# arkiven4/glow-tts

Measured on AMD Instinct MI355X. Metric: mel_frames_per_sec_train_step, higher is better.
Workload: dtype bf16; 1 GPU; configs/base.json, LJSpeech-shaped synthetic batches, B=32/GPU, T_x<=150, T_y<=800, bf16 GEMMs; batch_per_gpu=32, T_x=150, T_y=800, batches_rotated=8, padded_frames_per_gpu_step=25600, rows_layout=ragged, graphs_captured=6, parallelism=dp1 (utterance-sharded, RCCL gradient all-reduce, fp32 on the wire), launch=one HIP graph per step (one per ragged-row bucket, captured up front)

## Files before the change

### glow-tts_amd/csrc/conv_wgrad.hip

```cpp
#include <stdlib.h>
#include "common.h"
#include "mfma_frag.h"
#include "../../include/glowtts_hip.h"

namespace {

constexpr int SLAB_Q = 64;

typedef __attribute__((__vector_size__(4 * sizeof(short)))) short s16x4_t;

__device__ __forceinline__ unsigned lds_off(const void* p) { return (unsigned)reinterpret_cast<uintptr_t>(p); }

__device__ __forceinline__ bf16x8_t tr_frag(const unsigned char* p0, const unsigned char* p1) {
  const s16x4_t lo = __builtin_amdgcn_ds_read_tr16_b64_v4i16((__attribute__((address_space(3))) s16x4_t*)(uintptr_t)p0);
  const s16x4_t hi = __builtin_amdgcn_ds_read_tr16_b64_v4i16((__attribute__((address_space(3))) s16x4_t*)(uintptr_t)p1);
  typedef __attribute__((__vector_size__(8 * sizeof(short)))) short s16x8_t;
  s16x8_t v = {lo[0], lo[1], lo[2], lo[3], hi[0], hi[1], hi[2], hi[3]};
  return __builtin_bit_cast(bf16x8_t, v);
}

__device__ __forceinline__ void glds16(const void* src, unsigned dst_base) {
  unsigned keep;
  asm volatile("s_mov_b32 %0, m0\n\ts_mov_b32 m0, %2\n\ts_nop 0\n\t"
               "global_load_lds_dwordx4 %1, off\n\ts_mov_b32 m0, %0"
               : "=&s"(keep) : "v"(src), "s"(dst_base) : "memory");
}
template <int N> __device__ __forceinline__ void wait_vm() { asm volatile("s_waitcnt vmcnt(%0)" :: "n"(N) : "memory"); }

template <int TAPS, int NJ, int KB_, int NST_> struct WgGeo {
  static constexpr int KB = KB_, NST = NST_;
  static constexpr int XR = KB + TAPS - 1;
  static constexpr int XCH = 8 * NJ;
  static constexpr int YB = KB * 256, XB = XR * XCH * 16, STAGE = YB + XB;
  static constexpr int YI = KB / 16;
  static constexpr int NWX = XR * XCH / 4;
  static constexpr int XI = (NWX + 63) / 64;
  static constexpr int NLD = YI + XI;
  static constexpr int NB = TAPS * NJ;
  static constexpr int LDS = NST * STAGE;
  static_assert(KB % 16 == 0 && SLAB_Q % KB == 0, "stage rows");
  static_assert((XR * XCH) % 4 == 0, "X chunks split evenly over the waves");
  static_assert(LDS <= 80 * 1024, "two workgroups per CU");
  static_assert((NST - 2) * NLD <= 63, "vmcnt field");
  static_assert(TAPS == 1 || NJ == 1, "taps or channel groups");
};

template <int TAPS, int NJ, int KB_, int NST_>
__device__ __forceinline__ void wgrad_tile(
    const bf16_t* __restrict__ X, int ldx, const bf16_t* __restrict__ dY, int ldy,
    float* __restrict__ part, float* __restrict__ part_bias, int R, int Cin, int Cout, int slab_rows,
    int co0, int ci0, int slab, int co_begin, int Ncols)
{
  using G = WgGeo<TAPS, NJ, KB_, NST_>;
  constexpr int KB = G::KB, NST = G::NST, NB = G::NB;
  extern __shared__ __attribute__((aligned(1024))) unsigned char ring[];
  const int tid = threadIdx.x, lane = tid & 63, wave = __builtin_amdgcn_readfirstlane(tid >> 6);
  constexpr int padl = TAPS >> 1;
  const int mbeg = slab * slab_rows;
  const int mend = min(R, mbeg + slab_rows);
  const int nst = (mend - mbeg + KB - 1) / KB;
  const int wco = wave >> 1, wci = wave & 1;
  const bool do_bias = (ci0 == 0) && part_bias && wci == 0;

  f32x16_t acc[NB][2];
  float bsum[2] = {0.f, 0.f};
#pragma unroll
  for (int t = 0; t < NB; ++t)
#pragma unroll
    for (int j = 0; j < 2; ++j)
#pragma unroll
      for (int e = 0; e < 16; ++e) acc[t][j][e] = 0.0f;

  int yrow[G::YI], ycol[G::YI], xrow[G::XI], xcol[G::XI];
  bool xact[G::XI];
#pragma unroll
  for (int j = 0; j < G::YI; ++j) {
    const int L = j * 256 + tid, r = L >> 4, c = (L & 15) ^ ((r & 3) << 2);
    yrow[j] = r; ycol[j] = min(co0 + c * 8, Ncols - 8);
  }
#pragma unroll
  for (int j = 0; j < G::XI; ++j) {
    const int Lw = j * 64 + lane, L = wave * G::NWX + Lw, r = L / G::XCH, c = (L - r * G::XCH) ^ (((r >> 1) & 1) << 2);
    xact[j] = Lw < G::NWX;
    xrow[j] = r - padl; xcol[j] = min(ci0 + c * 8, Cin - 8);
  }
  const unsigned ring0 = lds_off(ring);

  auto issue = [&](int s, int sl_i) {
    const int mb = mbeg + s * KB;
    const unsigned slot = ring0 + (unsigned)sl_i * G::STAGE;
    const bool edge = (mb - padl < 0) || (mb + KB + padl > R) || (mb + KB > mend);
    if (!edge) {
#pragma unroll
      for (int j = 0; j < G::YI; ++j)
        glds16(dY + (size_t)(mb + yrow[j]) * ldy + ycol[j], slot + (unsigned)(j * 256 + wave * 64) * 16);
#pragma unroll
      for (int j = 0; j < G::XI; ++j)
        if (xact[j]) glds16(X + (ptrdiff_t)(mb + xrow[j]) * ldx + xcol[j], slot + G::YB + (unsigned)(wave * G::NWX + j * 64) * 16);
    } else {
      unsigned char* sl = ring + (size_t)sl_i * G::STAGE;
#pragma unroll
      for (int j = 0; j < G::YI; ++j) {
        const int m = mb + yrow[j];
        u32x4_t v = {0u, 0u, 0u, 0u};
        if (m < mend) v = *reinterpret_cast<const u32x4_t*>(dY + (size_t)m * ldy + ycol[j]);
        *reinterpret_cast<u32x4_t*>(sl + (size_t)(j * 256 + tid) * 16) = v;
      }
#pragma unroll
      for (int j = 0; j < G::XI; ++j) {
        const int m = mb + xrow[j];
        u32x4_t v = {0u, 0u, 0u, 0u};
        if (xact[j]) {
          if (m >= 0 && m < R) v = *reinterpret_cast<const u32x4_t*>(X + (size_t)m * ldx + xcol[j]);
          *reinterpret_cast<u32x4_t*>(sl + G::YB + (size_t)(wave * G::NWX + j * 64 + lane) * 16) = v;
        }
      }
    }
  };

  const int li = lane & 15, q = li >> 2, p = li & 3;
  const int colhalf = ((lane >> 4) & 1) * 16;
  const int h = lane >> 5;
  constexpr int NOX = TAPS < 4 ? TAPS : 4;
  int offA[2], offX[NOX];
#pragma unroll
  for (int i = 0; i < 2; ++i) {
    const int ch = wco * 8 + i * 4 + (colhalf >> 3) + (p >> 1);
    offA[i] = (8 * h + q) * 256 + ((ch ^ (q << 2)) << 4) + (p & 1) * 8;
  }
#pragma unroll
  for (int t = 0; t < NOX; ++t) {
    const int ch = wci * 4 + (colhalf >> 3) + (p >> 1);
    offX[t] = (8 * h + q) * (G::XCH * 16) + ((ch ^ ((((q + t) >> 1) & 1) << 2)) << 4) + (p & 1) * 8;
  }

  bf16x8_t af[2], bfg[NB];
  auto load_frags = [&](const unsigned char* yb, const unsigned char* xb, int ks) {
#pragma unroll
    for (int i = 0; i < 2; ++i) {
      const unsigned char* ya = yb + offA[i] + ks * 16 * 256;
      af[i] = tr_frag(ya, ya + 4 * 256);
    }
#pragma unroll
    for (int t = 0; t < TAPS; ++t)
#pragma unroll
      for (int j = 0; j < NJ; ++j) {
        const unsigned char* xa = xb + offX[t & 3] + (ks * 16 + t) * (G::XCH * 16) + j * 128;
        bfg[t * NJ + j] = tr_frag(xa, xa + 4 * (G::XCH * 16));
      }
  };
  auto mfmas = [&]() {
#pragma unroll
    for (int t = 0; t < NB; ++t)
#pragma unroll
      for (int i = 0; i < 2; ++i) acc[t][i] = __builtin_amdgcn_mfma_f32_32x32x16_bf16(af[i], bfg[t], acc[t][i], 0, 0, 0);
    if (do_bias) {
#pragma unroll
      for (int i = 0; i < 2; ++i) {
        const u32x4_t w4 = __builtin_bit_cast(u32x4_t, af[i]);
#pragma unroll
        for (int d = 0; d < 4; ++d) bsum[i] += __uint_as_float(w4[d] << 16) + __uint_as_float(w4[d] & 0xffff0000u);
      }
    }
  };

#pragma unroll 1
  for (int s = 0; s < NST - 1 && s < nst; ++s) issue(s, s);
  int cslot = 0, islot = NST - 1;
#pragma unroll 1
  for (int s = 0; s < nst; ++s) {
    const int after = min(nst - 1, s + NST - 2) - s;
    if (after >= NST - 2) wait_vm<(NST - 2) * G::NLD>();
    else wait_vm<0>();
    asm volatile("s_waitcnt lgkmcnt(0)\n\ts_barrier" ::: "memory");
    if (s + NST - 1 < nst) issue(s + NST - 1, islot);
    const unsigned char* yb = ring + (size_t)cslot * G::STAGE;
    const unsigned char* xb = yb + G::YB;
    cslot = cslot + 1 == NST ? 0 : cslot + 1;
    islot = islot + 1 == NST ? 0 : islot + 1;
#pragma unroll
    for (int ks = 0; ks < KB / 16; ++ks) {
      load_frags(yb, xb, ks);
      __builtin_amdgcn_sched_barrier(0);
      mfmas();
    }
  }

  const int r = lane & 31;
#pragma unroll
  for (int t = 0; t < TAPS; ++t)
#pragma unroll
    for (int j = 0; j < NJ; ++j) {
      const int ci = ci0 + j * 64 + wci * 32 + r;
#pragma unroll
      for (int i = 0; i < 2; ++i) {
        if (ci >= Cin) continue;
#pragma unroll
        for (int e = 0; e < 16; ++e) {
          const int co = co0 + wco * 64 + i * 32 + (e & 3) + 8 * (e >> 2) + 4 * h;
          if (co < Ncols) part[(((size_t)slab * TAPS + t) * Cout + co_begin + co) * Cin + ci] = acc[t * NJ + j][i][e];
        }
      }
    }
  if (do_bias) {
#pragma unroll
    for (int i = 0; i < 2; ++i) {
      const float tot = bsum[i] + __shfl_xor(bsum[i], 32);
      const int co = co0 + wco * 64 + i * 32 + r;
      if (h == 0 && co < Ncols) part_bias[(size_t)slab * Cout + co_begin + co] = tot;
    }
  }
}

template <int TAPS> struct WgSel;
template <> struct WgSel<5> { static constexpr int NJ = 1, KB = 64, NST = 3; };
template <> struct WgSel<3> { static constexpr int NJ = 1, KB = 64, NST = 3; };
template <> struct WgSel<1> { static constexpr int NJ = 3, KB = 32, NST = 3; };
template <int TAPS> using WgGeoT = WgGeo<TAPS, WgSel<TAPS>::NJ, WgSel<TAPS>::KB, WgSel<TAPS>::NST>;

template <int TAPS>
__global__ __launch_bounds__(256, 2) void gt_conv_wgrad_kernel(
    const bf16_t* __restrict__ X, int ldx, const bf16_t* __restrict__ dY, int ldy,
    float* __restrict__ part, float* __restrict__ part_bias, int R, int Cin, int Cout, int slab_rows)
{
  using S = WgSel<TAPS>;
  wgrad_tile<TAPS, S::NJ, S::KB, S::NST>(X, ldx, dY, ldy, part, part_bias, R, Cin, Cout, slab_rows,
                                         blockIdx.x * 128, blockIdx.y * 64 * S::NJ, blockIdx.z, 0, Cout);
}

template <int TAPS>
__global__ __launch_bounds__(256, 2) void gt_conv_wgrad_batched_kernel(
    const gt_wgrad_job* __restrict__ jobs, const gt_wgrad_tile* __restrict__ tiles)
{
  using S = WgSel<TAPS>;
  const gt_wgrad_tile t = tiles[blockIdx.x];
  const gt_wgrad_job j = jobs[t.job];
  wgrad_tile<TAPS, S::NJ, S::KB, S::NST>(static_cast<const bf16_t*>(j.X), j.ldx, static_cast<const bf16_t*>(j.dY), j.ldy,
                                         j.part, j.part_bias, j.R, j.Cin, j.Cout, j.slab_rows, t.co0, t.ci0, t.slab, j.co_begin, j.co_count);
}

template <int TAPS> static int wgrad_lds_attr()
{
  static int done = 0;
  if (!done) {
    if (hipFuncSetAttribute(reinterpret_cast<const void*>(&gt_conv_wgrad_kernel<TAPS>), hipFuncAttributeMaxDynamicSharedMemorySize, WgGeoT<TAPS>::LDS) != hipSuccess ||
        hipFuncSetAttribute(reinterpret_cast<const void*>(&gt_conv_wgrad_batched_kernel<TAPS>), hipFuncAttributeMaxDynamicSharedMemorySize, WgGeoT<TAPS>::LDS) != hipSuccess)
      return GT_E_LAUNCH;
    done = 1;
  }
  return 0;
}

constexpr int WNB_ROWS = 4;
__device__ __forceinline__ void weightnorm_bwd_row(
    const float* __restrict__ part, const float* __restrict__ part_bias, int S, const float* __restrict__ v,
    const float* __restrict__ g, const float* __restrict__ inv_norm, float* __restrict__ dv, float* __restrict__ dg,
    float* __restrict__ dbias, int Cout, int Cin, int taps, int accumulate, int co, float* dws)
{
  const int lane = threadIdx.x & 63, n = Cin * taps;
  if (dbias && lane == 0) {
    float sb = 0.f;
    for (int k = 0; k < S; ++k) sb += part_bias[(size_t)k * Cout + co];
    dbias[co] = accumulate ? dbias[co] + sb : sb;
  }
  const size_t sstride = (size_t)taps * Cout * Cin;
  for (int tap = 0; tap < taps; ++tap) {
    const float* pt = part + ((size_t)tap * Cout + co) * Cin;
    for (int ci = lane; ci < Cin; ci += 64) {
      const float* pp = pt + ci;
      float s0 = 0.f, s1 = 0.f, s2 = 0.f, s3 = 0.f;
      int k = 0;
      for (; k + 4 <= S; k += 4) {
        const float a0 = pp[(size_t)k * sstride], a1 = pp[(size_t)(k + 1) * sstride];
        const float a2 = pp[(size_t)(k + 2) * sstride], a3 = pp[(size_t)(k + 3) * sstride];
        s0 += a0; s1 += a1; s2 += a2; s3 += a3;
      }
      for (; k < S; ++k) s0 += pp[(size_t)k * sstride];
      dws[ci * taps + tap] = (s0 + s1) + (s2 + s3);
    }
  }
  __builtin_amdgcn_fence(__ATOMIC_RELEASE, "wavefront");
  __builtin_amdgcn_wave_barrier();
  __builtin_amdgcn_fence(__ATOMIC_ACQUIRE, "wavefront");
  const float* vr = v + (size_t)co * n;
  float* dr = dv + (size_t)co * n;
  if (!g) {
    for (int i = lane; i < n; i += 64) dr[i] = accumulate ? dr[i] + dws[i] : dws[i];
    return;
  }
  float dot = 0.f;
  for (int i = lane; i < n; i += 64) dot += dws[i] * vr[i];
  const float d = wave_sum(dot);
  const float inv = inv_norm[co], gg = g[co];
  if (lane == 0) dg[co] = accumulate ? dg[co] + d * inv : d * inv;
  const float a = gg * inv, bcoef = gg * d * inv * inv * inv;
  for (int i = lane; i < n; i += 64) {
    const float val = a * dws[i] - bcoef * vr[i];
    dr[i] = accumulate ? dr[i] + val : val;
  }
}

__global__ __launch_bounds__(64 * WNB_ROWS) void gt_weightnorm_bwd_kernel(
    const float* __restrict__ part, const float* __restrict__ part_bias, int S, const float* __restrict__ v,
    const float* __restrict__ g, const float* __restrict__ inv_norm, float* __restrict__ dv, float* __restrict__ dg,
    float* __restrict__ dbias, int Cout, int Cin, int taps, int accumulate)
{
  extern __shared__ float dws[];
  const int w = threadIdx.x >> 6, co = blockIdx.x * WNB_ROWS + w;
  if (co >= Cout) return;
  weightnorm_bwd_row(part, part_bias, S, v, g, inv_norm, dv, dg, dbias, Cout, Cin, taps, accumulate, co, dws + (size_t)w * Cin * taps);
}

__global__ __launch_bounds__(64 * WNB_ROWS) void gt_weightnorm_bwd_batched_kernel(const gt_wnb_job* __restrict__ jobs, int n_jobs, int total_rows,
                                                                                int max_row_elems)
{
  extern __shared__ float dws[];
  const int w = threadIdx.x >> 6, row = blockIdx.x * WNB_ROWS + w;
  if (row >= total_rows) return;
  int lo = 0, hi = n_jobs - 1;
  while (lo < hi) {
    const int mid = (lo + hi + 1) >> 1;
    if (jobs[mid].row_start <= row) lo = mid; else hi = mid - 1;
  }
  const gt_wnb_job j = jobs[lo];
  weightnorm_bwd_row(j.part, j.part_bias, j.S, j.v, j.g, j.inv_norm, j.dv, j.dg, j.dbias, j.Cout, j.Cin, j.taps,
                     j.accumulate, row - j.row_start, dws + (size_t)w * max_row_elems);
}

template <bool F32>
__global__ __launch_bounds__(256) void gt_colsum_kernel(const void* __restrict__ Y, int ldy, float* __restrict__ out,
                                                        int R, int N, int rows_per_block)
{
  __shared__ float red[4][64];
  const int c = blockIdx.x * 64 + (threadIdx.x & 63), ph = threadIdx.x >> 6;
  const int m0 = blockIdx.y * rows_per_block, m1 = min(R, m0 + rows_per_block);
  float s = 0.f;
  if (c < N) {
    for (int m = m0 + ph; m < m1; m += 4)
      s += F32 ? static_cast<const float*>(Y)[(size_t)m * ldy + c] : bf2f(static_cast<const bf16_t*>(Y)[(size_t)m * ldy + c]);
  }
  red[ph][threadIdx.x & 63] = s;
  __syncthreads();
  if (ph == 0 && c < N) atomicAdd(out + c, red[0][threadIdx.x] + red[1][threadIdx.x] + red[2][threadIdx.x] + red[3][threadIdx.x]);
}

}

extern "C" int gt_conv_wgrad_ci_tile(int taps)
{
  return taps == 1 ? 64 * WgSel<1>::NJ : taps == 3 ? 64 * WgSel<3>::NJ : taps == 5 ? 64 * WgSel<5>::NJ : 0;
}

extern "C" size_t gt_conv_wgrad_workspace_bytes(int R, int Cin, int Cout, int taps, int* slabs_out)
{
  if (R <= 0 || Cin <= 0 || Cout <= 0 || taps <= 0) { if (slabs_out) *slabs_out = 0; return 0; }
  const int cit = gt_conv_wgrad_ci_tile(taps) > 0 ? gt_conv_wgrad_ci_tile(taps) : 64;
  const int tiles = ((Cout + 127) / 128) * ((Cin + cit - 1) / cit);
  constexpr int target = 160;
  int S = (target + tiles - 1) / tiles;
  if (S > 16) S = 16;
  const int max_s = (R + SLAB_Q - 1) / SLAB_Q;
  if (S > max_s) S = max_s;
  if (S < 1) S = 1;
  if (slabs_out) *slabs_out = S;
  return ((size_t)S * taps * Cout * Cin + (size_t)S * Cout) * sizeof(float);
}

extern "C" int gt_conv_wgrad_bf16(const void* X, int ldx, const void* dY, int ldy, int R, int Cin, int Cout,
                                  int taps, void* workspace, size_t workspace_bytes, void* stream)
{
  if (R <= 0 || Cin <= 0 || Cout <= 0) return GT_E_INVAL;
  if (!X || !dY || !workspace) return GT_E_INVAL;
  if (taps != 1 && taps != 3 && taps != 5) return GT_E_UNSUPPORTED;
  if ((Cin & 7) || (Cout & 7) || (ldx & 7) || (ldy & 7)) return GT_E_ALIGN;
  if (((uintptr_t)X | (uintptr_t)dY) & 15) return GT_E_ALIGN;
  int S = 0;
  if (workspace_bytes < gt_conv_wgrad_workspace_bytes(R, Cin, Cout, taps, &S)) return GT_E_INVAL;
  const int slab_rows = (((R + S - 1) / S) + SLAB_Q - 1) / SLAB_Q * SLAB_Q;
  const int cit = gt_conv_wgrad_ci_tile(taps);
  const dim3 grid((Cout + 127) / 128, (Cin + cit - 1) / cit, S);
  hipStream_t st = static_cast<hipStream_t>(stream);
  const bf16_t* x = static_cast<const bf16_t*>(X); const bf16_t* dy = static_cast<const bf16_t*>(dY);
  float* part = static_cast<float*>(workspace);
  float* pb = part + (size_t)S * taps * Cout * Cin;
  if (wgrad_lds_attr<5>() || wgrad_lds_attr<3>() || wgrad_lds_attr<1>()) return GT_E_LAUNCH;
  if (taps == 5)      hipLaunchKernelGGL(gt_conv_wgrad_kernel<5>, grid, dim3(256), WgGeoT<5>::LDS, st, x, ldx, dy, ldy, part, pb, R, Cin, Cout, slab_rows);
  else if (taps == 3) hipLaunchKernelGGL(gt_conv_wgrad_kernel<3>, grid, dim3(256), WgGeoT<3>::LDS, st, x, ldx, dy, ldy, part, pb, R, Cin, Cout, slab_rows);
  else                hipLaunchKernelGGL(gt_conv_wgrad_kernel<1>, grid, dim3(256), WgGeoT<1>::LDS, st, x, ldx, dy, ldy, part, pb, R, Cin, Cout, slab_rows);
  return gt_launch_status(__func__);
}

extern "C" int gt_weightnorm_bwd(const void* workspace, int R, const float* v, const float* g, const float* inv_norm,
                                 float* dv, float* dg, float* dbias, int Cout, int Cin, int taps, int accumulate, void* stream)
{
  if (!workspace || !v || !dv || Cout <= 0 || Cin <= 0 || taps <= 0) return GT_E_INVAL;
  if (g && (!inv_norm || !dg)) return GT_E_INVAL;
  int S = 0;
  gt_conv_wgrad_workspace_bytes(R, Cin, Cout, taps, &S);
  const size_t lds = (size_t)WNB_ROWS * Cin * taps * sizeof(float);
  if (lds > 60 * 1024) return GT_E_UNSUPPORTED;
  const float* part = static_cast<const float*>(workspace);
  hipLaunchKernelGGL(gt_weightnorm_bwd_kernel, dim3((Cout + WNB_ROWS - 1) / WNB_ROWS), dim3(64 * WNB_ROWS), lds, static_cast<hipStream_t>(stream),
                     part, part + (size_t)S * taps * Cout * Cin, S, v, g, inv_norm, dv, dg, dbias, Cout, Cin, taps, accumulate);
  return gt_launch_status(__func__);
}

extern "C" int gt_conv_wgrad_batched(const void* jobs_device, const void* tiles_device, int n_tiles5, int n_tiles3,
                                     int n_tiles1, void* stream)
{
  if (!jobs_device || !tiles_device || n_tiles5 < 0 || n_tiles3 < 0 || n_tiles1 < 0) return GT_E_INVAL;
  hipStream_t st = static_cast<hipStream_t>(stream);
  const gt_wgrad_job* jobs = static_cast<const gt_wgrad_job*>(jobs_device);
  const gt_wgrad_tile* tiles = static_cast<const gt_wgrad_tile*>(tiles_device);
  if (wgrad_lds_attr<5>() || wgrad_lds_attr<3>() || wgrad_lds_attr<1>()) return GT_E_LAUNCH;
  if (n_tiles5) hipLaunchKernelGGL(gt_conv_wgrad_batched_kernel<5>, dim3(n_tiles5), dim3(256), WgGeoT<5>::LDS, st, jobs, tiles);
  if (n_tiles3) hipLaunchKernelGGL(gt_conv_wgrad_batched_kernel<3>, dim3(n_tiles3), dim3(256), WgGeoT<3>::LDS, st, jobs, tiles + n_tiles5);
  if (n_tiles1) hipLaunchKernelGGL(gt_conv_wgrad_batched_kernel<1>, dim3(n_tiles1), dim3(256), WgGeoT<1>::LDS, st, jobs, tiles + n_tiles5 + n_tiles3);
  return gt_launch_status(__func__);
}

extern "C" int gt_weightnorm_bwd_batched(const void* jobs_device, int n_jobs, int total_rows, int max_row_elems, void* stream)
{
  if (!jobs_device || n_jobs <= 0 || total_rows <= 0 || max_row_elems <= 0) return GT_E_INVAL;
  const size_t lds = (size_t)WNB_ROWS * max_row_elems * sizeof(float);
  if (lds > 60 * 1024) return GT_E_UNSUPPORTED;
  hipLaunchKernelGGL(gt_weightnorm_bwd_batched_kernel, dim3((total_rows + WNB_ROWS - 1) / WNB_ROWS), dim3(64 * WNB_ROWS), lds,
                     static_cast<hipStream_t>(stream), static_cast<const gt_wnb_job*>(jobs_device), n_jobs, total_rows, max_row_elems);
  return gt_launch_status(__func__);
}

extern "C" int gt_colsum(const void* Y, int ldy, int is_f32, float* out, int R, int N, void* stream)
{
  if (!Y || !out || R < 0 || N <= 0) return GT_E_INVAL;
  if (R == 0) return GT_OK;
  const int rows_per_block = 128;
  const dim3 grid((N + 63) / 64, (R + rows_per_block - 1) / rows_per_block);
  hipStream_t st = static_cast<hipStream_t>(stream);
  if (is_f32) hipLaunchKernelGGL(gt_colsum_kernel<true>,  grid, dim3(256), 0, st, Y, ldy, out, R, N, rows_per_block);
  else        hipLaunchKernelGGL(gt_colsum_kernel<false>, grid, dim3(256), 0, st, Y, ldy, out, R, N, rows_per_block);
  return gt_launch_status(__func__);
}
```

Before: 4.493 million mel-frames/s.

## Vectorize weight-norm backward with float4 slab reduction and LDS-staged v

Adds a wide path for the weight-norm backward row kernel. It sums split-K partial slabs with 16-byte vector loads using several accumulators, and stages both the reduced weight gradient and the v row in LDS, so the dot product and the dv update read LDS instead of global memory. The bias reduction switches to shuffles, and the batched kernel finds the job with a ballot/popcount scan instead of a binary search. LDS per row doubles, so the rows per block are now chosen dynamically to stay under the LDS cap, which can lower the number of rows per block and the occupancy for large rows.

```diff
diff --git a/glow-tts_amd/csrc/conv_wgrad.hip b/glow-tts_amd/csrc/conv_wgrad.hip
--- a/glow-tts_amd/csrc/conv_wgrad.hip
+++ b/glow-tts_amd/csrc/conv_wgrad.hip
@@ -300,31 +300,211 @@
   }
 }
 
-__global__ __launch_bounds__(64 * WNB_ROWS) void gt_weightnorm_bwd_kernel(
+constexpr int WNF_P = 4;
+typedef float wnf4_t __attribute__((ext_vector_type(4)));
+__device__ __forceinline__ wnf4_t wnf_ld4(const float* p) { return *(const __attribute__((address_space(1))) wnf4_t*)(uintptr_t)p; }
+__device__ __forceinline__ float wnf_ld1(const float* p) { return *(const __attribute__((address_space(1))) float*)(uintptr_t)p; }
+__device__ __forceinline__ void wnf_st4(float* p, wnf4_t x) { *(__attribute__((address_space(1))) wnf4_t*)(uintptr_t)p = x; }
+
+__device__ __forceinline__ float wnf_dv(float a, float dw, float bcoef, float x)
+{
+#pragma clang fp contract(off)
+  const float l = a * dw, r = bcoef * x;
+  return l - r;
+}
+
+template <int NS>
+__device__ __forceinline__ void wnf_slabs_few(const float* const (&pp)[WNF_P], size_t sstride, wnf4_t (&t)[WNF_P])
+{
+  asm volatile("; %0 slab(s) per pass" :: "n"(NS) : "memory");
+  wnf4_t a[WNF_P][NS];
+#pragma unroll
+  for (int p = 0; p < WNF_P; ++p)
+#pragma unroll
+    for (int q = 0; q < NS; ++q) a[p][q] = wnf_ld4(pp[p] + (size_t)q * sstride);
+#pragma unroll
+  for (int p = 0; p < WNF_P; ++p) {
+    wnf4_t s0 = 0.f;
+#pragma unroll
+    for (int q = 0; q < NS; ++q) s0 += a[p][q];
+    t[p] = (s0 + 0.f) + (0.f + 0.f);
+  }
+}
+
+__device__ __forceinline__ void weightnorm_bwd_row16(
+    const float* __restrict__ part, const float* __restrict__ part_bias, int S, const float* __restrict__ v,
+    const float* __restrict__ g, const float* __restrict__ inv_norm, float* __restrict__ dv, float* __restrict__ dg,
+    float* __restrict__ dbias, int Cout, int Cin, int taps, int accumulate, int co, float* dws, float* vs)
+{
+  const int lane = threadIdx.x & 63, n = Cin * taps, nch = n >> 2;
+  const unsigned c4 = (unsigned)Cin >> 2;
+  const size_t sstride = (size_t)taps * Cout * Cin;
+  const float* vr = v + (size_t)co * n;
+  float* dr = dv + (size_t)co * n;
+  float pb, odb, inv, gg, odg;
+  if (dbias) {
+    pb = wnf_ld1(part_bias + (size_t)max(min(lane, S - 1), 0) * Cout + co);
+    if (accumulate) odb = wnf_ld1(dbias + co);
+  }
+  if (g) {
+    inv = wnf_ld1(inv_norm + co); gg = wnf_ld1(g + co);
+    if (accumulate) odg = wnf_ld1(dg + co);
+  }
+  wnf4_t od[WNF_P];
+  if (accumulate) {
+#pragma unroll
+    for (int p = 0; p < WNF_P; ++p) od[p] = wnf_ld4(dr + 4 * min(64 * p + lane, nch - 1));
+  }
+  for (int c0 = 0; c0 < nch; c0 += 64 * WNF_P) {
+    const float* pp[WNF_P]; int o[WNF_P]; wnf4_t vv[WNF_P], t[WNF_P];
+#pragma unroll
+    for (int p = 0; p < WNF_P; ++p) {
+      const unsigned c = (unsigned)min(c0 + 64 * p + lane, nch - 1);
+      const unsigned tap = c / c4, ci = (c - tap * c4) * 4;
+      pp[p] = part + ((size_t)tap * Cout + co) * Cin + ci;
+      o[p] = (int)(ci * taps + tap);
+    }
+    if (g) {
+#pragma unroll
+      for (int p = 0; p < WNF_P; ++p) vv[p] = wnf_ld4(vr + 4 * min(c0 + 64 * p + lane, nch - 1));
+    }
+    if (S <= 2) {
+      if (S == 1) wnf_slabs_few<1>(pp, sstride, t);
+      else        wnf_slabs_few<2>(pp, sstride, t);
+#pragma unroll
+      for (int p = 0; p < WNF_P; ++p) {
+        if (c0 + 64 * p + lane >= nch) continue;
+        float* d = dws + o[p];
+        d[0] = t[p].x; d[taps] = t[p].y; d[2 * taps] = t[p].z; d[3 * taps] = t[p].w;
+      }
+    } else {
+#pragma unroll 1
+      for (int p = 0; p < WNF_P; ++p) {
+        const int cp = c0 + 64 * p + lane;
+        const unsigned c = (unsigned)min(cp, nch - 1);
+        const unsigned tap = c / c4, ci = (c - tap * c4) * 4;
+        const float* q = part + ((size_t)tap * Cout + co) * Cin + ci;
+        wnf4_t s0 = 0.f, s1 = 0.f, s2 = 0.f, s3 = 0.f;
+        int k = 0;
+        for (; k + 4 <= S; k += 4) {
+          const wnf4_t a0 = wnf_ld4(q + (size_t)k * sstride), a1 = wnf_ld4(q + (size_t)(k + 1) * sstride);
+          const wnf4_t a2 = wnf_ld4(q + (size_t)(k + 2) * sstride), a3 = wnf_ld4(q + (size_t)(k + 3) * sstride);
+          s0 += a0; s1 += a1; s2 += a2; s3 += a3;
+        }
+        for (; k < S; ++k) s0 += wnf_ld4(q + (size_t)k * sstride);
+        const wnf4_t r = (s0 + s1) + (s2 + s3);
+        if (cp < nch) {
+          float* d = dws + ci * taps + tap;
+          d[0] = r.x; d[taps] = r.y; d[2 * taps] = r.z; d[3 * taps] = r.w;
+        }
+      }
+    }
+    if (g) {
+#pragma unroll
+      for (int p = 0; p < WNF_P; ++p) {
+        const int c = c0 + 64 * p + lane;
+        if (c < nch) *reinterpret_cast<wnf4_t*>(vs + 4 * c) = vv[p];
+      }
+    }
+  }
+  if (dbias) {
+    float sb = 0.f;
+    for (int k0 = 0; k0 < S; k0 += 64) {
+      if (k0) pb = wnf_ld1(part_bias + (size_t)min(k0 + lane, S - 1) * Cout + co);
+      const int m = min(64, S - k0);
+      for (int k = 0; k < m; ++k) sb += __shfl(pb, k);
+    }
+    if (lane == 0) dbias[co] = accumulate ? odb + sb : sb;
+  }
+  __builtin_amdgcn_fence(__ATOMIC_RELEASE, "wavefront");
+  __builtin_amdgcn_wave_barrier();
+  __builtin_amdgcn_fence(__ATOMIC_ACQUIRE, "wavefront");
+  float a = 1.f, bcoef = 0.f;
+  if (g) {
+    float dot = 0.f;
+    for (int i = lane; i < n; i += 64) dot = __builtin_fmaf(dws[i], vs[i], dot);
+    const float d = wave_sum(dot);
+    if (lane == 0) dg[co] = accumulate ? __builtin_fmaf(d, inv, odg) : d * inv;
+    a = gg * inv; bcoef = gg * d * inv * inv * inv;
+  }
+  for (int c0 = 0; c0 < nch; c0 += 64 * WNF_P) {
+    if (c0 && accumulate) {
+#pragma unroll
+      for (int p = 0; p < WNF_P; ++p) od[p] = wnf_ld4(dr + 4 * min(c0 + 64 * p + lane, nch - 1));
+    }
+#pragma unroll
+    for (int p = 0; p < WNF_P; ++p) {
+      const int c = c0 + 64 * p + lane;
+      if (c >= nch) continue;
+      wnf4_t val = *reinterpret_cast<const wnf4_t*>(dws + 4 * c);
+      if (g) {
+        const wnf4_t x = *reinterpret_cast<const wnf4_t*>(vs + 4 * c);
+        val.x = wnf_dv(a, val.x, bcoef, x.x); val.y = wnf_dv(a, val.y, bcoef, x.y);
+        val.z = wnf_dv(a, val.z, bcoef, x.z); val.w = wnf_dv(a, val.w, bcoef, x.w);
+      }
+      if (accumulate) { val.x = od[p].x + val.x; val.y = od[p].y + val.y; val.z = od[p].z + val.z; val.w = od[p].w + val.w; }
+      wnf_st4(dr + 4 * c, val);
+    }
+  }
+}
+
+__device__ __forceinline__ void weightnorm_bwd_dispatch(
+    const float* __restrict__ part, const float* __restrict__ part_bias, int S, const float* __restrict__ v,
+    const float* __restrict__ g, const float* __restrict__ inv_norm, float* __restrict__ dv, float* __restrict__ dg,
+    float* __restrict__ dbias, int Cout, int Cin, int taps, int accumulate, int co, float* strip, int strip_elems)
+{
+  const bool wide = !(Cin & 3) && !((reinterpret_cast<uintptr_t>(part) | reinterpret_cast<uintptr_t>(v) | reinterpret_cast<uintptr_t>(dv)) & 15);
+  if (wide) {
+    weightnorm_bwd_row16(part, part_bias, S, v, g, inv_norm, dv, dg, dbias, Cout, Cin, taps, accumulate, co, strip, strip + strip_elems);
+  } else {
+    weightnorm_bwd_row(part, part_bias, S, v, g, inv_norm, dv, dg, dbias, Cout, Cin, taps, accumulate, co, strip);
+    __builtin_amdgcn_s_waitcnt(0x0070);
+  }
+}
+
+__global__ __launch_bounds__(64 * WNB_ROWS, 3) void gt_weightnorm_bwd_kernel(
     const float* __restrict__ part, const float* __restrict__ part_bias, int S, const float* __restrict__ v,
     const float* __restrict__ g, const float* __restrict__ inv_norm, float* __restrict__ dv, float* __restrict__ dg,
     float* __restrict__ dbias, int Cout, int Cin, int taps, int accumulate)
 {
-  extern __shared__ float dws[];
-  const int w = threadIdx.x >> 6, co = blockIdx.x * WNB_ROWS + w;
+  extern __shared__ __attribute__((aligned(16))) float dws[];
+  const int w = threadIdx.x >> 6, co = blockIdx.x * (blockDim.x >> 6) + w;
   if (co >= Cout) return;
-  weightnorm_bwd_row(part, part_bias, S, v, g, inv_norm, dv, dg, dbias, Cout, Cin, taps, accumulate, co, dws + (size_t)w * Cin * taps);
-}
-
-__global__ __launch_bounds__(64 * WNB_ROWS) void gt_weightnorm_bwd_batched_kernel(const gt_wnb_job* __restrict__ jobs, int n_jobs, int total_rows,
+  const int strip = (Cin * taps + 3) & ~3;
+  weightnorm_bwd_dispatch(part, part_bias, S, v, g, inv_norm, dv, dg, dbias, Cout, Cin, taps, accumulate, co, dws + (size_t)w * 2 * strip, strip);
+}
+
+__global__ __launch_bounds__(64 * WNB_ROWS, 3) void gt_weightnorm_bwd_batched_kernel(const gt_wnb_job* __restrict__ jobs, int n_jobs, int total_rows,
                                                                                 int max_row_elems)
 {
-  extern __shared__ float dws[];
-  const int w = threadIdx.x >> 6, row = blockIdx.x * WNB_ROWS + w;
+  extern __shared__ __attribute__((aligned(16))) float dws[];
+  const int w = threadIdx.x >> 6, lane = threadIdx.x & 63, row = blockIdx.x * (blockDim.x >> 6) + w;
   if (row >= total_rows) return;
-  int lo = 0, hi = n_jobs - 1;
-  while (lo < hi) {
-    const int mid = (lo + hi + 1) >> 1;
-    if (jobs[mid].row_start <= row) lo = mid; else hi = mid - 1;
-  }
+  int cnt = 0;
+  for (int i0 = 0; i0 < n_jobs; i0 += 256) {
+    int rs[4];
+#pragma unroll
+    for (int u = 0; u < 4; ++u) {
+      const int i = i0 + 64 * u + lane;
+      rs[u] = jobs[min(i, n_jobs - 1)].row_start;
+    }
+#pragma unroll
+    for (int u = 0; u < 4; ++u) cnt += __popcll(__ballot(i0 + 64 * u + lane < n_jobs && rs[u] <= row));
+  }
+  const int lo = __builtin_amdgcn_readfirstlane(cnt > 0 ? cnt - 1 : 0);
   const gt_wnb_job j = jobs[lo];
-  weightnorm_bwd_row(j.part, j.part_bias, j.S, j.v, j.g, j.inv_norm, j.dv, j.dg, j.dbias, j.Cout, j.Cin, j.taps,
-                     j.accumulate, row - j.row_start, dws + (size_t)w * max_row_elems);
+  const int strip = (max_row_elems + 3) & ~3;
+  weightnorm_bwd_dispatch(j.part, j.part_bias, j.S, j.v, j.g, j.inv_norm, j.dv, j.dg, j.dbias, j.Cout, j.Cin, j.taps,
+                          j.accumulate, row - j.row_start, dws + (size_t)w * 2 * strip, strip);
+}
+
+constexpr size_t WNB_LDS_MAX = 60 * 1024;
+static size_t wnb_lds(int rows, int max_row_elems) { return (size_t)rows * 2 * ((max_row_elems + 3) & ~3) * sizeof(float); }
+static int wnb_rows(int max_row_elems)
+{
+  int rows = WNB_ROWS;
+  while (rows > 1 && wnb_lds(rows, max_row_elems) > WNB_LDS_MAX) --rows;
+  return rows;
 }
 
 template <bool F32>
@@ -397,10 +577,11 @@
   if (g && (!inv_norm || !dg)) return GT_E_INVAL;
   int S = 0;
   gt_conv_wgrad_workspace_bytes(R, Cin, Cout, taps, &S);
-  const size_t lds = (size_t)WNB_ROWS * Cin * taps * sizeof(float);
-  if (lds > 60 * 1024) return GT_E_UNSUPPORTED;
+  if ((size_t)WNB_ROWS * Cin * taps * sizeof(float) > WNB_LDS_MAX) return GT_E_UNSUPPORTED;
+  const int rows = wnb_rows(Cin * taps);
+  const size_t lds = wnb_lds(rows, Cin * taps);
   const float* part = static_cast<const float*>(workspace);
-  hipLaunchKernelGGL(gt_weightnorm_bwd_kernel, dim3((Cout + WNB_ROWS - 1) / WNB_ROWS), dim3(64 * WNB_ROWS), lds, static_cast<hipStream_t>(stream),
+  hipLaunchKernelGGL(gt_weightnorm_bwd_kernel, dim3((Cout + rows - 1) / rows), dim3(64 * rows), lds, static_cast<hipStream_t>(stream),
                      part, part + (size_t)S * taps * Cout * Cin, S, v, g, inv_norm, dv, dg, dbias, Cout, Cin, taps, accumulate);
   return gt_launch_status(__func__);
 }
@@ -422,9 +603,10 @@
 extern "C" int gt_weightnorm_bwd_batched(const void* jobs_device, int n_jobs, int total_rows, int max_row_elems, void* stream)
 {
   if (!jobs_device || n_jobs <= 0 || total_rows <= 0 || max_row_elems <= 0) return GT_E_INVAL;
-  const size_t lds = (size_t)WNB_ROWS * max_row_elems * sizeof(float);
-  if (lds > 60 * 1024) return GT_E_UNSUPPORTED;
-  hipLaunchKernelGGL(gt_weightnorm_bwd_batched_kernel, dim3((total_rows + WNB_ROWS - 1) / WNB_ROWS), dim3(64 * WNB_ROWS), lds,
+  if ((size_t)WNB_ROWS * max_row_elems * sizeof(float) > WNB_LDS_MAX) return GT_E_UNSUPPORTED;
+  const int rows = wnb_rows(max_row_elems);
+  const size_t lds = wnb_lds(rows, max_row_elems);
+  hipLaunchKernelGGL(gt_weightnorm_bwd_batched_kernel, dim3((total_rows + rows - 1) / rows), dim3(64 * rows), lds,
                      static_cast<hipStream_t>(stream), static_cast<const gt_wnb_job*>(jobs_device), n_jobs, total_rows, max_row_elems);
   return gt_launch_status(__func__);
 }
```

After: 4.564 million mel-frames/s, median of 6. +1.6%, better.
